# Giovannibriglia/ContinuousBayesianNetwork

Hardware: AMD Instinct MI355X
Metric: marginal queries/sec + achieved HBM GB/s, 20-node d=32 DAG, 65k-batch VE (higher is better)
Workload: dtype f32; 1 GPU; chain20_d32: BayesianNetwork.infer target X19, evidence on the other 19 nodes, N_max=32; queries_per_gpu=65536, global_batch=65536, parallelism=query-shard x1

## Files before the change

### continuousbayesiannetwork_amd/_native.py

```python
from __future__ import annotations

import ctypes
import os

import torch

from . import _buildstamp

_HERE = os.path.dirname(os.path.abspath(__file__))
_DEFAULT_LIB = os.path.join(_HERE, "libcbn_amd.so")


def lib_path() -> str:
    alt = os.environ.get("CBN_LIB_PATH")
    if alt and os.environ.get("CBN_DIAG") == "1":
        return alt
    return _DEFAULT_LIB


LIB_PATH = lib_path()

ABI_VERSION = 5
CBN_MAX_PARENTS = 8
CBN_MAX_DIRECT_PARENTS = 32
# ... 118 lines not shown
    "cbn_plan_max_words": (ctypes.c_int32, [ctypes.c_void_p]),
    "cbn_plan_run_fold": (ctypes.c_int, [ctypes.c_void_p, ctypes.c_int64, ctypes.c_void_p, ctypes.c_int32,
                                         ctypes.c_void_p, ctypes.c_void_p, ctypes.c_void_p, ctypes.c_int64,
                                         ctypes.c_void_p, ctypes.c_int32, ctypes.c_int32, ctypes.c_void_p]),
    "cbn_plan_run_argmax": (ctypes.c_int, [ctypes.c_void_p, ctypes.c_int64, ctypes.c_void_p, ctypes.c_int32,
                                           ctypes.c_void_p, ctypes.c_void_p, ctypes.c_void_p, ctypes.c_void_p,
                                           ctypes.c_void_p, ctypes.c_int32, ctypes.c_void_p]),
    "cbn_plan_argmax_scratch": (ctypes.c_int64, [ctypes.c_void_p, ctypes.c_int64]),
    "cbn_row_argmax": (ctypes.c_int, [ctypes.c_void_p, ctypes.c_int64, ctypes.c_int32, ctypes.c_void_p,
                                      ctypes.c_void_p, ctypes.c_void_p, ctypes.c_void_p, ctypes.c_void_p]),
    "cbn_plan_create_param": (ctypes.c_int, [ctypes.POINTER(ParamFactor), ctypes.c_int32, ctypes.c_int32,
                                             ctypes.POINTER(ctypes.c_void_p)]),
    "cbn_param_eval": (ctypes.c_int, [ctypes.POINTER(ParamModel), ctypes.c_void_p, ctypes.c_int64, ctypes.c_int32,
                                      ctypes.c_void_p, ctypes.c_int32, ctypes.c_void_p, ctypes.c_void_p]),
    "cbn_hash_build": (ctypes.c_int, [ctypes.c_void_p, ctypes.c_void_p, ctypes.c_int64, ctypes.c_void_p,
                                      ctypes.c_void_p, ctypes.c_int64, ctypes.c_void_p]),
    "cbn_cpd_ref_eval": (ctypes.c_int, [ctypes.POINTER(CpdRef), ctypes.c_void_p, ctypes.c_int64, ctypes.c_void_p,
                                        ctypes.c_void_p]),
    "cbn_plan_create_direct": (ctypes.c_int, [ctypes.POINTER(DirectFactor), ctypes.c_int32, ctypes.c_int32,
                                              ctypes.POINTER(ctypes.c_void_p)]),
}
CBN_RUN_BUILD_TABLES = 1
CBN_RUN_TIMED = 2
CBN_RUN_TWO_PASS = 4
CBN_RUN_RAW = 8
CBN_E_LIMIT = -3
CBN_E_UNSUPPORTED = -4
CBN_E_TIMEOUT = -5
CBN_PLAN_FAST, CBN_PLAN_LDS, CBN_PLAN_PAIRED, CBN_PLAN_STAGED = 1, 2, 4, 8
CBN_PLAN_FUSED, CBN_PLAN_PARAMETRIC, CBN_PLAN_VPL2, CBN_PLAN_DIRECT = 16, 32, 64, 128
CBN_PLAN_COLS = 256
CBN_PLAN_SLOTS = 512
CBN_PLAN_ARGMAX = 1024
CBN_E_ARG = -1

EXPORTED_SYMBOLS = tuple(_SIGNATURES)

_lib = None


class NativeError(RuntimeError):
    pass


def _check_stamp(path: str, digest: str) -> None:
    got = _buildstamp.read_stamp(path)
    if got != digest:
        raise NativeError(
            f"{path} was not built from this tree's sources (stamp {got or 'missing'} != {digest[:16]}...): "
            "rebuild it with `python -c 'import __graft_entry__ as g; g.build()'`")


def load() -> ctypes.CDLL:
    global _lib
    if _lib is None:
        if not os.path.exists(LIB_PATH):
            raise NativeError(
                f"{LIB_PATH} is missing: build it with `python -c 'import __graft_entry__ as g; g.build()'` "
                "(no CPU fallback exists for the HIP inference path)")
        if LIB_PATH == _DEFAULT_LIB:
            _check_stamp(LIB_PATH, _buildstamp.lib_digest())
        lib = ctypes.CDLL(LIB_PATH)
        for name, (res, args) in _SIGNATURES.items():
            fn = getattr(lib, name)
            fn.restype = res
            fn.argtypes = args
# ... 53 lines not shown
```

### continuousbayesiannetwork_amd/csrc/cbn_infer.hip

```cpp

#include <hip/hip_runtime.h>

#include <algorithm>
#include <cstdarg>
#include <cstdint>
#include <cstdio>
#include <cstdlib>
#include <cstring>
#include <string>
#include <type_traits>
#include <vector>

#include <unistd.h>

#include "cbn_internal.h"

using namespace cbn;

namespace {
thread_local std::string g_err;
}

namespace {
const bool g_diag = [] {
// ... 247 lines not shown
__device__ __forceinline__ void store_wt(__amdgpu_buffer_rsrc_t r, int off, float4 v) {
    u32x4_t x = {__float_as_uint(v.x), __float_as_uint(v.y), __float_as_uint(v.z), __float_as_uint(v.w)};
#ifndef CBN_STORE_AUX
#define CBN_STORE_AUX 16
#endif
    __builtin_amdgcn_raw_buffer_store_b128(x, r, off, 0, CBN_STORE_AUX);
}

__device__ __forceinline__ int4 sload_int4(const void* p) {
    const cint_t* q = reinterpret_cast<const cint_t*>(reinterpret_cast<uintptr_t>(p));
    return make_int4(q[0], q[1], q[2], q[3]);
}

constexpr int kChunkBytes = kWave * 16;
template <int K>
__device__ __forceinline__ void lds_dma_group(const float4* gp, float4* lp) {
    __builtin_amdgcn_global_load_lds((gbl_void_t*)gp, (lds_void_t*)lp, 16, 0, 0);
    if (K > 1) __builtin_amdgcn_global_load_lds((gbl_void_t*)gp, (lds_void_t*)lp, 16, kChunkBytes, 0);
    if (K > 2) __builtin_amdgcn_global_load_lds((gbl_void_t*)gp, (lds_void_t*)lp, 16, 2 * kChunkBytes, 0);
    if (K > 3) __builtin_amdgcn_global_load_lds((gbl_void_t*)gp, (lds_void_t*)lp, 16, 3 * kChunkBytes, 0);
}
__device__ __forceinline__ void lds_dma_segment(const float4* gl, float4* lds, int a, int b) {
    const float4* gp = gl + a * kWave;
    float4* lp = lds + a * kWave;
    int n = b - a;
    for (; n >= 4; n -= 4, gp += 4 * kWave, lp += 4 * kWave) lds_dma_group<4>(gp, lp);
    if (n & 2) {
        lds_dma_group<2>(gp, lp);
        gp += 2 * kWave;
        lp += 2 * kWave;
    }
    if (n & 1) lds_dma_group<1>(gp, lp);
}
__device__ __forceinline__ void lds_dma_copy(const float* __restrict__ g, float4* lds, int n4,
                                             int nw = kQueryThreads / kWave) {
    const int lane = threadIdx.x & (kWave - 1);
    const int wave = __builtin_amdgcn_readfirstlane(threadIdx.x / kWave);
    const int nchunk = (n4 + kWave - 1) / kWave;
    const int run = (nchunk + nw - 1) / nw;
    const int r0 = wave * run;
    const int len = nchunk - r0 < run ? nchunk - r0 : run;
    if (len <= 0 || !CBN_OK_OR(n4 > 0 && wave < nw, 0)) return;
    int start = r0 + (int)(blockIdx.x % (unsigned)nchunk);
    if (start >= nchunk) start -= nchunk;
    const int over = start + len - nchunk;
    const int tail = n4 & (kWave - 1);
    const float4* gl = reinterpret_cast<const float4*>(g) + lane;
    const bool masked = over >= 0 && tail != 0;
    lds_dma_segment(gl, lds, start, (over >= 0 ? nchunk : start + len) - (masked ? 1 : 0));
    if (masked && lane < tail) lds_dma_group<1>(gl + (nchunk - 1) * kWave, lds + (nchunk - 1) * kWave);
    if (over > 0) lds_dma_segment(gl, lds, 0, over);
}

__global__ void k_cpd_scatter(const int32_t* __restrict__ cell, const float* __restrict__ prob,
                              long long n_rows, float* __restrict__ cpd) {
    for (long long r = blockIdx.x * (long long)blockDim.x + threadIdx.x; r < n_rows;
         r += (long long)gridDim.x * blockDim.x)
        cpd[cell[r]] = prob[r];
}

__global__ void k_cpd_normalize(float* __restrict__ cpd, long long n_pcells, int card) {
    for (long long c = blockIdx.x * (long long)blockDim.x + threadIdx.x; c < n_pcells;
         c += (long long)gridDim.x * blockDim.x) {
        float* row = cpd + c * card;
        double s = 0.0;
        for (int v = 0; v < card; ++v) s += (double)row[v];
        const float den = (float)s + 1e-10f;
        for (int v = 0; v < card; ++v) row[v] = row[v] / den;
    }
}

__global__ void k_cpd_eval(const float* __restrict__ cpd, int n_cols, ColPtrs cols,
                           const float* __restrict__ pts, long long n_pts, float* __restrict__ out) {
    for (long long i = blockIdx.x * (long long)blockDim.x + threadIdx.x; i < n_pts;
         i += (long long)gridDim.x * blockDim.x) {
        long long off = 0;
// ... 1124 lines not shown
#pragma unroll
            for (int i = 0; i < NV; ++i) acc0[i] = acc[i];
        }
        round_epilogue<VPL, MODE>(acc, col, l, L, valid, valid, q, N, out, maxv, lmax, !first, fq, am);
        __builtin_amdgcn_s_waitcnt(0xC07F);
        __builtin_amdgcn_wave_barrier();
        if (first) CBN_STAMP(6);
        first = false;
    }
    CBN_STAMP(7);
    if (MODE == kModeMax || MODE == kModeRaw) publish_block_max(lmax, wmax, max_out, n_max, lane, wid, tid, nthr);
    if (MODE == kModeFused) {
        maxv = fused_block_max(lmax, wmax, sync, epoch, max_out, lane, wid, nthr CBN_STAMP_ARG);
        if (fq0 >= 0) store_row_div<VPL>(out + fq0 * N, col, acc0, maxv);
        if (fq >= 0) store_row_div<VPL>(out + fq * N, col, acc, maxv);
        CBN_STAMP(10);
    }
}

constexpr int kSR = 256;
constexpr int kSQ = 128;
constexpr int kSU = 4;

struct FoldJob {
    float* rows;
    const unsigned* words;
    long long n4;
    long long chunk;
    int n_words;
};
constexpr int kFoldK = 2;
constexpr int kFoldW = 4;

template <int MODE>
__global__ void __launch_bounds__(kQueryThreads)
k_query_staged(const float* __restrict__ gimage, int image_floats, int rec_off, int nf, int zero_off, long long Q,
               long long per, unsigned* __restrict__ sync, unsigned epoch, const unsigned* __restrict__ max_in,
               int n_max, unsigned* __restrict__ max_out, float* __restrict__ out, FoldJob fold,
               FPtrsT<kFastPtrsSmall> fp, ArgmaxOut am) {
    CBN_STAMP_INIT;
    constexpr int N = 32;
    extern __shared__ __attribute__((aligned(16))) float4 smem4[];
    float* simg = reinterpret_cast<float*>(smem4);
    const int T = (nf + 2) >> 1;
    const int S = (T + 1) >> 1;
    const int nsl = 4 * (S + 1);
    int* offs = reinterpret_cast<int*>(simg + image_floats);
    float* wmax = reinterpret_cast<float*>(offs + 2 * kSR * nsl);
    const int tid = threadIdx.x;
    const int lane = tid & (kWave - 1);
    const int wid = __builtin_amdgcn_readfirstlane(tid / kWave);
    const long long q0 = (long long)blockIdx.x * per;
    const long long q1 = q0 + per < Q ? q0 + per : Q;
    const int nunits = nf * (kSR / kSQ);
    const FastRec* grec = reinterpret_cast<const FastRec*>(gimage + rec_off);
    const int one_off = zero_off + 64;

    float x[kSU][2] = {};
    auto stage_load = [&](long long qr, auto ksu, int gw, int GW) {
        constexpr int KSU = decltype(ksu)::value;
        uintptr_t pk[KSU];
#pragma unroll
        for (int k = 0; k < KSU; ++k) {
            const int u = gw + k * GW;
            pk[k] = reinterpret_cast<uintptr_t>(fp.p[((u / (kSR / kSQ)) & 31) * kFastObs]);
        }
#pragma unroll
        for (int k = 0; k < KSU; ++k) {
            const int u = gw + k * GW;
            if (u < nunits) {
                const float* col = reinterpret_cast<const float*>(pk[k] & ~(kTagMore | kTagNone));
#pragma unroll
                for (int h = 0; h < 2; ++h) {
                    const long long q = qr + (u % (kSR / kSQ)) * kSQ + h * kWave + lane;
                    x[k][h] = gload(col, (pk[k] & kTagNone) ? 0 : (q < q1 ? q : q0));
                }
            }
        }
    };
    auto stage_store = [&](long long qr, int buf, auto ksu, int gw, int GW) {
        constexpr int KSU = decltype(ksu)::value;
        int* ob = offs + buf * kSR * nsl;
        int4 rk[KSU];
#pragma unroll
        for (int k = 0; k < KSU; ++k) {
            const int u = gw + k * GW;
            rk[k] = sload_int4(grec + (u < nunits ? u / (kSR / kSQ) : 0));
        }
#pragma unroll
        for (int k = 0; k < KSU; ++k) {
            const int u = gw + k * GW;
// ... 19 lines not shown
                        if (n_obs > 1) {
                            const long long q = qr + ql;
#pragma unroll
                            for (int p = 1; p < kFastObs; ++p)
                                if (p < n_obs) xs[p] = gload(fp.p[f * kFastObs + p], q < q1 ? q : q0);
                        }
                        int row = 0;
                        bool ok = true;
#pragma unroll
                        for (int p = 0; p < kFastObs; ++p) {
                            if (p < n_obs) {
                                const int card = r.card[p] & (kDenseBit - 1);
                                const float xv = xs[p];
                                int i;
                                if (r.card[p] & kDenseBit) {
                                    i = (int)xv;
                                    i = (xv >= 0.f && xv < (float)card && (float)i == xv) ? i : -1;
                                } else {
                                    i = bsearch_eq(gimage + r.dom_off[p], card, xv);
                                }
                                ok &= i >= 0;
                                row = row * card + (i < 0 ? 0 : i);
                            }
                        }
                        o = ok ? r.table_off + row * 64 : zoff;
                    }
                    ob[ql * nsl + f + ((ql >> 1) & 1)] = o;
                }
            }
        }
    };

    long long qr = q0;
#ifndef CBN_ABL_NODMA
    lds_dma_copy(gimage, smem4, image_floats / 4);
#endif
#ifndef CBN_ABL_NOSTAGE
    if (qr < q1) stage_load(qr, std::integral_constant<int, kSU>{}, wid, kQueryThreads / kWave);
#endif
    CBN_STAMP(1);
    if (tid < kSR) {
        const int d = (tid >> 1) & 1;
        for (int j = 0; j < nsl; ++j) {
            const int f = j - d;
            if (f < 0 || f >= nf) {
                const int o = one_off + (f & 1) * 32;
                offs[tid * nsl + j] = o;
                offs[kSR * nsl + tid * nsl + j] = o;
            }
        }
    }
    if (qr < q1)
        stage_store(qr, 0, std::integral_constant<int, kSU>{}, wid, kQueryThreads / kWave);
    CBN_STAMP(2);
    __syncthreads();
    CBN_STAMP(3);
    float4 fv[kFoldK];
    unsigned fw[kFoldW];
    const long long fb = (long long)blockIdx.x * fold.chunk;
    const long long fe = fb + fold.chunk < fold.n4 ? fb + fold.chunk : fold.n4;
    if (MODE == kModeRaw && fold.rows) {
        const float4* r4 = reinterpret_cast<const float4*>(fold.rows);
#pragma unroll
        for (int k = 0; k < kFoldK; ++k) {
            const long long i = fb + tid + k * kQueryThreads;
            fv[k] = i < fe ? r4[i] : make_float4(0.f, 0.f, 0.f, 0.f);
        }
#pragma unroll
        for (int k = 0; k < kFoldW; ++k) {
            const int w = lane + k * kWave;
            fw[k] = w < fold.n_words ? fold.words[w] : 0u;
        }
    }

    const int qi = lane >> 2;
    const int l = lane & 3;
    const int h0 = qi & 1;
    const int clo = (l + 4 * h0) * 4, chi = (l + 4 * (h0 ^ 1)) * 4;
    float lmax = 0.f;
    float maxv = 1.f;
    if (MODE == kModeWrite) maxv = batch_max(max_in, n_max, max_out, lane, tid);
    float acc[8];
    long long fq = -1;
    int buf = 0;
    const bool wt_raw = MODE == kModeRaw && fold.rows != nullptr;
    const __amdgpu_buffer_rsrc_t orsrc =
        rows_rsrc((MODE == kModeFused || wt_raw) ? out + q0 * N : nullptr,
                  (MODE == kModeFused || wt_raw) ? (q1 - q0) * (long long)(N * 4) : 0);
    for (; qr < q1; qr += kSR, buf ^= 1) {
        const long long qn = qr + kSR;
        if (MODE != kModeFused && qn < q1) stage_load(qn, std::integral_constant<int, kSU>{}, wid, kQueryThreads / kWave);
        const int ql = wid * 16 + qi;
        const long long q = qr + ql;
        const int* my = offs + buf * kSR * nsl + ql * nsl;
#pragma unroll
        for (int i = 0; i < 8; ++i) acc[i] = 1.f;
        auto mul_step = [&](const float4& r0, const float4& r1, const float4& r2, const float4& r3) {
            acc[0] *= r0.x; acc[1] *= r0.y; acc[2] *= r0.z; acc[3] *= r0.w;
            acc[4] *= r1.x; acc[5] *= r1.y; acc[6] *= r1.z; acc[7] *= r1.w;
            acc[0] *= r2.x; acc[1] *= r2.y; acc[2] *= r2.z; acc[3] *= r2.w;
            acc[4] *= r3.x; acc[5] *= r3.y; acc[6] *= r3.z; acc[7] *= r3.w;
        };
        auto load_step = [&](int oa, int ob, float4& r0, float4& r1, float4& r2, float4& r3) {
            r0 = *reinterpret_cast<const float4*>(simg + oa + clo);
            r1 = *reinterpret_cast<const float4*>(simg + oa + chi);
            r2 = *reinterpret_cast<const float4*>(simg + ob + clo);
            r3 = *reinterpret_cast<const float4*>(simg + ob + chi);
        };
        typedef float vf4 __attribute__((ext_vector_type(4)));
        typedef const volatile __attribute__((address_space(3))) vf4 lds_vf4;
        auto vld = [&](int o) {
            const vf4 v = *(lds_vf4*)(simg + o);
            return make_float4(v.x, v.y, v.z, v.w);
        };
        auto vload_step = [&](int oa, int ob, float4& r0, float4& r1, float4& r2, float4& r3) {
            r0 = vld(oa + clo);
            r1 = vld(oa + chi);
            r2 = vld(ob + clo);
            r3 = vld(ob + chi);
        };
        float4 A0, A1, A2, A3, B0, B1, B2, B3;
        int4 on = *reinterpret_cast<const int4*>(my);
        vload_step(on.x, on.y, A0, A1, A2, A3);
        vload_step(on.z, on.w, B0, B1, B2, B3);
// ... 12 lines not shown
            mul_step(A0, A1, A2, A3);
            load_step(on.x, on.y, A0, A1, A2, A3);
            mul_step(B0, B1, B2, B3);
            load_step(on.z, on.w, B0, B1, B2, B3);
            on = *reinterpret_cast<const int4*>(my + 4 * min(sp + 2, S));
        }
#endif
        CBN_STAMP(5);
        if (MODE == kModeArgmax) {
            const int colv[2] = {clo, chi};
            argmax_store<2>(acc, colv, l, 4, q < q1, q, am);
        }
        if (q < q1) {
            if (MODE == kModeFused) fq = q;
            if (MODE == kModeRaw && wt_raw) {
                const int ob = (int)(q - q0) * (N * 4);
                store_wt(orsrc, ob + clo * 4, make_float4(acc[0], acc[1], acc[2], acc[3]));
                store_wt(orsrc, ob + chi * 4, make_float4(acc[4], acc[5], acc[6], acc[7]));
            } else if (MODE == kModeWrite || MODE == kModeRaw) {
                const float dv = MODE == kModeWrite ? maxv : 1.f;
                float* o = out + q * N;
                *reinterpret_cast<float4*>(o + clo) = MODE == kModeWrite
                    ? make_float4(acc[0] / dv, acc[1] / dv, acc[2] / dv, acc[3] / dv)
                    : make_float4(acc[0], acc[1], acc[2], acc[3]);
                *reinterpret_cast<float4*>(o + chi) = MODE == kModeWrite
                    ? make_float4(acc[4] / dv, acc[5] / dv, acc[6] / dv, acc[7] / dv)
                    : make_float4(acc[4], acc[5], acc[6], acc[7]);
            }
            if (MODE != kModeWrite && MODE != kModeArgmax)
#pragma unroll
                for (int i = 0; i < 8; ++i) lmax = fmaxf(lmax, acc[i]);
        }
        if (MODE != kModeFused && qn < q1) {
            stage_store(qn, buf ^ 1, std::integral_constant<int, kSU>{}, wid, kQueryThreads / kWave);
            __syncthreads();
        }
    }
    CBN_STAMP(6);
    if (MODE == kModeRaw && fold.rows) {
        unsigned m = 0;
#pragma unroll
        for (int k = 0; k < kFoldW; ++k) m = max(m, fw[k]);
        m = wave_max_u(m);
        const double y = 1.0 / (double)__uint_as_float(m);
        float4* r4 = reinterpret_cast<float4*>(fold.rows);
        const __amdgpu_buffer_rsrc_t frsrc = rows_rsrc(fold.rows + fb * 4, fe > fb ? (fe - fb) * 16 : 0);
#pragma unroll
        for (int k = 0; k < kFoldK; ++k) {
            const long long i = fb + tid + k * kQueryThreads;
            if (i < fe)
                store_wt(frsrc, (int)(i - fb) * 16,
                         make_float4((float)((double)fv[k].x * y), (float)((double)fv[k].y * y),
                                     (float)((double)fv[k].z * y), (float)((double)fv[k].w * y)));
        }
        for (long long i = fb + tid + kFoldK * kQueryThreads; i < fe; i += kQueryThreads) {
            const float4 v = r4[i];
            r4[i] = make_float4((float)((double)v.x * y), (float)((double)v.y * y), (float)((double)v.z * y),
                                (float)((double)v.w * y));
        }
    }
    if (MODE == kModeMax || MODE == kModeRaw) publish_block_max(lmax, wmax, max_out, n_max, lane, wid, tid, kQueryThreads);
    if (MODE == kModeFused) {
        lmax = wave_max_nonneg(lmax);
        if (lane == 0) wmax[wid] = lmax;
        __syncthreads();
        CBN_STAMP(7);
        if (wid == 0) {
            const float bm = wave_max_nonneg(lane < kQueryThreads / kWave ? wmax[lane] : 0.f);
#ifdef CBN_ABL_NOBAR
            const unsigned gm = __float_as_uint(bm);
#else
            const unsigned gm = slot_barrier_max(sync, epoch, bm);
#endif
            if (lane == 0) {
                wmax[0] = __uint_as_float(gm);
                if (blockIdx.x == 0 && max_out) *max_out = gm;
            }
        }
        CBN_STAMP(8);
        __syncthreads();
        CBN_STAMP(9);
        maxv = wmax[0];
        if (fq >= 0) {
            const double y = 1.0 / (double)maxv;
            float o[8];
#pragma unroll
            for (int i = 0; i < 8; ++i) o[i] = (float)((double)acc[i] * y);
            const int ob = (int)(fq - q0) * (N * 4);
            store_wt(orsrc, ob + clo * 4, make_float4(o[0], o[1], o[2], o[3]));
            store_wt(orsrc, ob + chi * 4, make_float4(o[4], o[5], o[6], o[7]));
        }
        CBN_STAMP(10);
        CBN_CLOCK_END;
    }
}

__device__ __forceinline__ unsigned max_words(const unsigned* __restrict__ w, int n) {
    const int lane = threadIdx.x & (kWave - 1);
    unsigned m = 0;
    int i = lane;
    for (; i + 15 * kWave < n; i += 16 * kWave) {
        unsigned t[16];
#pragma unroll
        for (int k = 0; k < 16; ++k) t[k] = w[i + k * kWave];
#pragma unroll
        for (int k = 0; k < 16; ++k) m = max(m, t[k]);
    }
    for (; i + 3 * kWave < n; i += 4 * kWave) {
        unsigned t[4];
#pragma unroll
        for (int k = 0; k < 4; ++k) t[k] = w[i + k * kWave];
#pragma unroll
        for (int k = 0; k < 4; ++k) m = max(m, t[k]);
    }
    for (; i < n; i += kWave) m = max(m, w[i]);
    return wave_max_u(m);
}

__device__ __forceinline__ float4 div4(float4 v, float m) {
    v.x = v.x / m;
    v.y = v.y / m;
    v.z = v.z / m;
    v.w = v.w / m;
    return v;
}

template <int U>
// ... 160 lines not shown
}

size_t slots_lds_bytes(long long lds_tab_floats, int ns, int nf, int QB) {
    const size_t nf4 = (size_t)((nf + 3) & ~3);
    const size_t SQ = (size_t)slots_sidx_stride(kQueryThreads / QB);
    size_t b = (size_t)lds_tab_floats * 4 + (size_t)ns * sizeof(QSlot) + (size_t)nf * sizeof(ColRec) +
               (size_t)((ns + 1) & ~1) * sizeof(void*) + ((((size_t)ns * SQ + 7) & ~size_t(7)) * 2) +
               (size_t)QB * nf4 * 4 + (kQueryThreads / kWave) * 4 + 64;
    return (b + 15) & ~size_t(15);
}

template <int VPL, bool LDS, int MODE, int NP>
void launch_fast_np(const cbn_plan* p, unsigned blocks, hipStream_t s, const EvPtrs& ev, long long Q, int L,
                    unsigned epoch, const unsigned* max_in, int n_max, unsigned* max_out, float* out,
                    const ArgmaxOut& am) {
    hipLaunchKernelGGL((k_query_fast<VPL, LDS, MODE, NP>), dim3(blocks), dim3(kQueryThreads), p->fast_lds_bytes, s,
                       p->rec_off, p->nf, p->ns, p->d_image, p->image_floats, fast_ptrs<NP>(p, ev), Q,
                       (Q + blocks - 1) / blocks, p->N, p->RS, L, p->paired ? 1 : 0, p->d_sync, epoch, max_in, n_max,
                       max_out, out, p->lds_tab_floats, p->lds_tab_mask[0], p->lds_tab_mask[1], am);
}

template <int VPL, bool LDS, int MODE>
void launch_fast_k(const cbn_plan* p, unsigned blocks, hipStream_t s, const EvPtrs& ev, long long Q, int L,
                   unsigned epoch, const unsigned* max_in, int n_max, unsigned* max_out, float* out,
                   const FoldJob* fold = nullptr, const ArgmaxOut* amp = nullptr) {
    const ArgmaxOut am = amp ? *amp : ArgmaxOut{nullptr, nullptr, nullptr, nullptr};
    if (p->staged) {
        FoldJob fj;
        memset(&fj, 0, sizeof(fj));
        if (fold && fold->rows && fold->n4 > 0) {
            fj = *fold;
            fj.chunk = (fj.n4 + blocks - 1) / blocks;
        }
        hipLaunchKernelGGL((k_query_staged<MODE>), dim3(blocks), dim3(kQueryThreads), p->staged_lds_bytes, s,
                           p->d_image, p->image_floats, p->rec_off + p->prefix * kRecFloats, p->nf - p->prefix,
                           p->zero_off, Q, (Q + blocks - 1) / blocks, p->d_sync, epoch, max_in, n_max, max_out, out,
                           fj, fast_ptrs<kFastPtrsSmall>(p, ev, p->prefix), am);
        return;
    }
    if (p->slots) {
        const int QBs = kQueryThreads / L;
        long long per = (Q + blocks - 1) / blocks;
        int coal = per > 2LL * QBs && !diag_env("CBN_SLOTS_NO_COAL") ? 1 : 0;
        if (diag_env("CBN_SLOTS_COAL")) coal = 1;
        for (int i = 0; i < p->ns; ++i) coal &= (reinterpret_cast<uintptr_t>(ev.p[i]) & 15) == 0 ? 1 : 0;
        if (coal) per = (per + 3) & ~3LL;
        hipLaunchKernelGGL((k_query_slots<VPL, MODE>), dim3(blocks), dim3(kQueryThreads), p->fast_lds_bytes, s, p->nf,
                           p->ns, p->d_image, p->rec_off + p->nf * kRecFloats, p->d_crec, slot_ptrs(p, ev), Q, per,
                           p->N, L, p->d_sync, epoch, max_in, n_max, max_out, out, p->lds_tab_floats,
                           p->lds_tab_mask[0], p->lds_tab_mask[1], coal, am);
        return;
    }
    if (p->cols) {
        auto k = (p->ns + L - 1) / L <= 16 ? k_query_cols<VPL, LDS, MODE, 16> : k_query_cols<VPL, LDS, MODE, 40>;
        hipLaunchKernelGGL(k, dim3(blocks), dim3(kQueryThreads), p->fast_lds_bytes, s,
                           p->rec_off, p->nf, p->ns, p->d_image, p->image_floats, slot_ptrs(p, ev), Q,
                           (Q + blocks - 1) / blocks, p->N, p->RS, L, p->d_sync, epoch, max_in, n_max, max_out, out,
                           p->lds_tab_floats, p->d_crec, am);
        return;
    }
    if (p->nf * kFastObs <= kFastPtrsSmall)
        launch_fast_np<VPL, LDS, MODE, kFastPtrsSmall>(p, blocks, s, ev, Q, L, epoch, max_in, n_max, max_out, out, am);
    else
        launch_fast_np<VPL, LDS, MODE, kFastPtrs>(p, blocks, s, ev, Q, L, epoch, max_in, n_max, max_out, out, am);
}

template <int VPL, bool LDS, int MODE>
const void* fast_kernel_fn(int nf, bool cols = false, int slots_per_lane = 0) {
    if (cols)
        return slots_per_lane <= 16 ? reinterpret_cast<const void*>(&k_query_cols<VPL, LDS, MODE, 16>)
// ... 549 lines not shown
            }
        }
    }
    int vpl = 0, Lf = 0;
    if (fast) {
        int want = 2;
        if (const char* e = diag_env("CBN_FAST_VPL")) want = atoi(e);
        for (int c : {2, 1}) {
            if (c > want || (N / 4) % c) continue;
            const int Lc = N / (4 * c);
            if (Lc <= kWave && (kWave % Lc) == 0) { vpl = c; Lf = Lc; break; }
        }
        fast = vpl > 0;
    }
    if (fast) {
        const int nf4 = (n_factors + 3) & ~3;
        const size_t side = (size_t)kFastPtrs * sizeof(void*) +
                            (size_t)(kQueryThreads / kWave) * (kWave / Lf) * nf4 * 4 + (kQueryThreads / kWave) * 4 + 64;
        const bool lds_ok = img_bytes + side <= (size_t)kLdsBudget;
        if (!lds_ok && P->use_lds) fast = false;
        if (!P->use_lds && (size_t)P->lds_tab_floats * 4 + (size_t)n_factors * kRecFloats * 4 + side > (size_t)kLdsBudget)
            fast = false;
        if (fast) {
            P->fast = true;
            P->vpl = vpl;
            P->paired = paired && vpl == 2 && P->use_lds;
            const int st_T = (n_factors - P->prefix + 2) >> 1, st_S = (st_T + 1) >> 1;
            const size_t st_bytes =
                img_bytes + (size_t)2 * kSR * (4 * (st_S + 1)) * 4 + (kQueryThreads / kWave) * 4 + 64;
            if (P->paired && (n_factors - P->prefix) * kFastObs <= kFastPtrsSmall && st_bytes <= (size_t)kLdsBudget &&
                !diag_env("CBN_NO_STAGED")) {
                P->staged = true;
                P->staged_lds_bytes = (st_bytes + 15) & ~size_t(15);
                for (const void* fn : {reinterpret_cast<const void*>(&k_query_staged<kModeMax>),
                                       reinterpret_cast<const void*>(&k_query_staged<kModeWrite>),
                                       reinterpret_cast<const void*>(&k_query_staged<kModeFused>),
                                       reinterpret_cast<const void*>(&k_query_staged<kModeRaw>),
                                       reinterpret_cast<const void*>(&k_query_staged<kModeArgmax>)})
                    (void)hipFuncSetAttribute(fn, hipFuncAttributeMaxDynamicSharedMemorySize, kLdsBudget);
            }
            P->fast_lds_bytes =
                ((P->use_lds ? img_bytes : (size_t)P->lds_tab_floats * 4 + (size_t)n_factors * kRecFloats * 4) + side +
                 15) & ~size_t(15);
            if (!P->staged && !P->paired && Lf <= 2 && ns <= kFastPtrsSmall && n_factors <= kWave &&
                !diag_env("CBN_NO_COLS")) {
                std::vector<ColRec> cr;
                bool ok_c = col_records(recs, slot_card, ns, RS, P->use_lds, lds_mask, cr);
                const size_t QBc = (size_t)kQueryThreads / Lf;
                const size_t cols_bytes =
                    ((P->use_lds ? img_bytes
                                 : (size_t)P->lds_tab_floats * 4 + ((size_t)n_factors * kRecFloats + (size_t)ns * 4) * 4) +
                     (size_t)((ns + 1) & ~1) * sizeof(void*) + (((size_t)ns * QBc + 1) & ~size_t(1)) * 2 +
                     (kQueryThreads / kWave) * 4 + 64 + 16 + (size_t)N * 4 + 15) & ~size_t(15);
                if (ok_c && cols_bytes <= (size_t)kLdsBudget) {
                    ok_c = hipMalloc(&P->d_crec, sizeof(ColRec) * n_factors) == hipSuccess &&
                           hipMemcpy(P->d_crec, cr.data(), sizeof(ColRec) * n_factors, hipMemcpyHostToDevice) ==
                               hipSuccess;
                    if (!ok_c) {
                        cbn_plan_destroy(P);
                        return set_err(CBN_E_HIP, "cbn_plan_create: column records upload failed");
                    }
                    P->cols = true;
                    P->fast_lds_bytes = cols_bytes;
                }
            }
            if (!P->staged && !P->paired && !P->cols && !P->use_lds && Lf > 2 && ns <= kFastPtrsSmall &&
                n_factors <= 128 && !diag_env("CBN_NO_SLOTS")) {
                std::vector<ColRec> cr;
                bool ok_s = col_records(recs, slot_card, ns, RS, false, lds_mask, cr);
                for (int f = 0; f < n_factors; ++f)
                    ok_s = ok_s && (long long)recs[f].table_off + (long long)fac[f].rows * RS < (1LL << 31);
                const size_t sb = slots_lds_bytes(P->lds_tab_floats, ns, n_factors, kQueryThreads / Lf);
                if (ok_s && sb <= (size_t)kLdsBudget) {
                    if (hipMalloc(&P->d_crec, sizeof(ColRec) * n_factors) != hipSuccess ||
                        hipMemcpy(P->d_crec, cr.data(), sizeof(ColRec) * n_factors, hipMemcpyHostToDevice) !=
                            hipSuccess) {
                        cbn_plan_destroy(P);
                        return set_err(CBN_E_HIP, "cbn_plan_create: slot records upload failed");
                    }
                    P->slots = true;
                    P->fast_lds_bytes = sb;
                }
            }
            P->fast_blocks_per_cu = 2 * P->fast_lds_bytes <= (size_t)kLdsBudget ? 2 : 1;
            if (P->slots)
                if (const char* e = diag_env("CBN_SLOTS_BPC")) P->fast_blocks_per_cu = atoi(e) == 2 ? 2 : 1;
            P->max_slots = std::min(num_cu() * P->fast_blocks_per_cu, kMaxSlots);
            if (hipMemcpy(P->d_image + rec_off, recs.data(), sizeof(FastRec) * n_factors, hipMemcpyHostToDevice) !=
                    hipSuccess ||
                (ns > 0 && hipMemcpy(P->d_image + rec_off + (long long)n_factors * kRecFloats, qs.data(),
                                     sizeof(QSlot) * ns, hipMemcpyHostToDevice) != hipSuccess)) {
                cbn_plan_destroy(P);
                return set_err(CBN_E_HIP, "cbn_plan_create: fast records upload failed");
            }
            if (!diag_env("CBN_NO_FUSED")) {
                allow_fast_lds<1, true, kModeFused>(kLdsBudget);
                allow_fast_lds<2, true, kModeFused>(kLdsBudget);
                allow_fast_lds<1, false, kModeFused>(kLdsBudget);
                allow_fast_lds<2, false, kModeFused>(kLdsBudget);
                int nb = 0;
                const int spl = (ns + Lf - 1) / Lf;
                const void* fn = with_variant(P, [&](auto v, auto lds) {
                    if (P->staged) return reinterpret_cast<const void*>(&k_query_staged<kModeFused>);
                    if (P->slots) return reinterpret_cast<const void*>(&k_query_slots<v.value, kModeFused>);
                    return fast_kernel_fn<v.value, lds.value, kModeFused>(n_factors, P->cols, spl);
                });
                const size_t lb = P->staged ? P->staged_lds_bytes : P->fast_lds_bytes;
                if (hipOccupancyMaxActiveBlocksPerMultiprocessor(&nb, fn, kQueryThreads, lb) == hipSuccess && nb >= 1)
                    P->fused_ok = true;
            }
        }
    }
    if (!P->staged && P->prefix) {
        P->prefix = 0;
        P->prefix_rows = 0;
    }
    allow_lds<4, true, false>(kLdsBudget); allow_lds<4, true, true>(kLdsBudget);
    allow_lds<1, true, false>(kLdsBudget); allow_lds<1, true, true>(kLdsBudget);
    allow_lds<4, false, false>(kLdsBudget); allow_lds<4, false, true>(kLdsBudget);
    allow_lds<1, false, false>(kLdsBudget); allow_lds<1, false, true>(kLdsBudget);
    if (!P->d_fac || !P->d_slots || !P->d_build || !P->d_image || !P->d_sync) {
        cbn_plan_destroy(P);
        return set_err(CBN_E_HIP, "cbn_plan_create: internal error, plan buffer missing");
    }
    *plan = P;
    return CBN_OK;
}

int cbn_plan_destroy(cbn_plan* plan) {
    if (!plan) return CBN_OK;
    for (int i = 0; i < cbn_plan::kRing; ++i)
        for (int k = 0; k < 3; ++k)
            if (plan->ev[i][k]) (void)hipEventDestroy(plan->ev[i][k]);
    if (plan->d_fac) (void)hipFree(plan->d_fac);
    if (plan->d_crec) (void)hipFree(plan->d_crec);
    if (plan->d_slots) (void)hipFree(plan->d_slots);
// ... 200 lines not shown
    EvPtrs ev;
    CBN_TRY(pack_evidence(plan, evidence, n_evidence, n_queries, ev));
    return launch_mode<kModeArgmax>(plan, n_queries, ev, nullptr, 0, nullptr, nullptr, s, nullptr, &am);
}

int cbn_plan_status(cbn_plan* plan, int32_t* status) {
    if (!plan || !status) return set_err(CBN_E_ARG, "cbn_plan_status: bad arguments");
    unsigned v = 0;
    HIP_TRY(hipMemcpy(&v, plan->d_sync + 2, sizeof(unsigned), hipMemcpyDeviceToHost));
    *status = (int32_t)v;
    if (plan->h_status) __atomic_store_n(plan->h_status, 0u, __ATOMIC_RELEASE);
    return CBN_OK;
}

int cbn_plan_check(cbn_plan* plan) {
    if (!plan) return set_err(CBN_E_ARG, "cbn_plan_check: null plan");
    if (plan->h_status && __atomic_load_n(plan->h_status, __ATOMIC_ACQUIRE)) {
        __atomic_store_n(plan->h_status, 0u, __ATOMIC_RELEASE);
        return set_err(CBN_E_TIMEOUT, "a single-launch call of this plan timed out in its grid barrier (another "
                                      "stream held CUs its blocks needed): its rows are NaN");
    }
    return CBN_OK;
}

int64_t cbn_plan_fused_capacity(const cbn_plan* plan) { return plan ? fused_capacity(plan) : 0; }

int32_t cbn_plan_flags(const cbn_plan* plan) {
    if (!plan) return 0;
    return (plan->fast ? CBN_PLAN_FAST : 0) | (plan->use_lds ? CBN_PLAN_LDS : 0) |
           (plan->paired ? CBN_PLAN_PAIRED : 0) | (plan->staged ? CBN_PLAN_STAGED : 0) |
           (plan->fused_ok ? CBN_PLAN_FUSED : 0) | (plan->param ? CBN_PLAN_PARAMETRIC : 0) |
           (plan->vpl == 2 ? CBN_PLAN_VPL2 : 0) | (plan->direct ? CBN_PLAN_DIRECT : 0) |
           (plan->cols ? CBN_PLAN_COLS : 0) | (plan->slots ? CBN_PLAN_SLOTS : 0) |
           (argmax_native(plan) ? CBN_PLAN_ARGMAX : 0);
}

int32_t cbn_plan_max_words(const cbn_plan* plan) {
    if (plan && plan->param) return param_max_words(plan->param);
    if (plan && plan->direct) return direct_max_words(plan->direct);
    return plan && plan->fast ? plan->max_slots : 0;
}

int cbn_scale(float* out, int64_t n, const uint32_t* max_bits, int32_t n_max, void* stream) {
    if (n < 0 || n_max < 1 || (n > 0 && (!out || !max_bits))) return set_err(CBN_E_ARG, "cbn_scale: bad arguments");
    if (n == 0) return CBN_OK;
    if (reinterpret_cast<uintptr_t>(out) % 16) return set_err(CBN_E_ARG, "cbn_scale: out must be 16-B aligned");
    return launch_scale(out, (long long)n, max_bits, (int)n_max, nullptr, reinterpret_cast<hipStream_t>(stream));
}

namespace {
int scale_blocks_per_cu() {
    static int v = [] {
        const char* e = diag_env("CBN_SCALE_BLOCKS_PER_CU");
        const int x = e ? atoi(e) : 0;
        return x >= 1 && x <= 16 ? x : 1;
    }();
    return v;
}
}

int cbn_scale_batch(float* const* outs, const int64_t* n_elems, int32_t n_batches, const uint32_t* max_bits,
                    int32_t n_max, void* stream) {
    if (n_batches < 0 || n_batches > kScaleBatch || n_max < 1 || (n_batches > 0 && (!outs || !n_elems || !max_bits)))
        return set_err(CBN_E_ARG, "cbn_scale_batch: bad arguments (at most %d batches)", kScaleBatch);
    if (n_batches == 0) return CBN_OK;
    ScaleBatch sb;
    memset(&sb, 0, sizeof(sb));
// ... 46 lines not shown
```

### continuousbayesiannetwork_amd/csrc/cbn_internal.h

```cpp
#ifndef CBN_INTERNAL_H
#define CBN_INTERNAL_H

#include <hip/hip_runtime.h>

#include <cstdint>

#include "../../include/cbn_amd.h"

namespace cbn {

constexpr int kWave = 64;
constexpr int kLdsBudget = 160 * 1024;
constexpr int kFastPtrs = 416;

constexpr int kSyncLine = 32;
constexpr int kHostStatusWordOff = 8;
constexpr int kOneWordOff = 12;
constexpr int kMaxSlots = 1024;
constexpr int kSlotWordOff = kSyncLine;
constexpr int kMaxWordOff = kSlotWordOff + 2 * kMaxSlots;
constexpr int kSyncWords = kMaxWordOff + kMaxSlots;

struct DevFactor;
struct QSlot;
// ... 16 lines not shown
               uint32_t* max_bits, float* out, int32_t flags, hipStream_t s);
int direct_build_consts(DirectPlan* dp, hipStream_t s);
void direct_destroy(DirectPlan* dp);
int direct_max_words(const DirectPlan* dp);

}

struct cbn_plan {
    int nf = 0;
    int ns = 0;
    int N = 0;
    int vec = 1;
    int L = 1;
    int CH = 1;
    cbn::DevFactor* d_fac = nullptr;
    int* d_crec = nullptr;
    cbn::QSlot* d_slots = nullptr;
    cbn::BuildItem* d_build = nullptr;
    int n_build = 0;
    int build_units = 0;
    float* d_image = nullptr;
    unsigned* d_sync = nullptr;
    bool fast = false;
    int fast_slot[cbn::kFastPtrs];
    static constexpr int kRing = 512;
    hipEvent_t ev[kRing][3] = {};
    int ev_n = 0;
    int rec_off = 0;
    int RS = 1;
    int vpl = 1;
    bool paired = false;
    bool staged = false;
    size_t staged_lds_bytes = 0;
    bool cols = false;
    bool slots = false;
    int zero_off = -1;
    int prefix = 0;
    int prefix_offs[9] = {};
    int prefix_rows = 0;
    unsigned* h_status = nullptr;
    unsigned fused_epoch = 0;
    bool fused_ok = false;
    size_t fast_lds_bytes = 0;
    int lds_tab_floats = 0;
    unsigned long long lds_tab_mask[2] = {0, 0};
    int fast_blocks_per_cu = 1;
    int max_slots = 0;
    int image_floats = 0;
    int table_floats = 0;
    bool use_lds = false;
    size_t lds_bytes = 0;
    int blocks_per_cu = 1;
    cbn::ParamPlan* param = nullptr;
    cbn::DirectPlan* direct = nullptr;
};

#endif
```

### include/cbn_amd.h

```cpp
#ifndef CBN_AMD_H
#define CBN_AMD_H

#include <stdint.h>

#ifdef __cplusplus
extern "C" {
#endif

#define CBN_AMD_ABI_VERSION 5

#define CBN_MAX_PARENTS 8
#define CBN_MAX_EVIDENCE 256

#define CBN_OK 0
#define CBN_E_ARG -1
#define CBN_E_HIP -2
#define CBN_E_LIMIT -3
#define CBN_E_UNSUPPORTED -4
#define CBN_E_TIMEOUT -5

#define CBN_FACTOR_SCALAR 0
#define CBN_FACTOR_SHARED 1
#define CBN_FACTOR_QUERY 2

// ... 83 lines not shown

int cbn_scale(float* out, int64_t n, const uint32_t* max_bits, int32_t n_max, void* stream);
int cbn_scale_batch(float* const* outs, const int64_t* n_elems, int32_t n_batches, const uint32_t* max_bits,
                    int32_t n_max, void* stream);
int cbn_plan_run_fold(cbn_plan* plan, int64_t n_queries, const float* const* evidence, int32_t n_evidence,
                      uint32_t* max_bits, float* out, float* fold_rows, int64_t fold_n_elems,
                      const uint32_t* fold_words, int32_t fold_n_words, int32_t flags, void* stream);
int cbn_plan_status(cbn_plan* plan, int32_t* status);


int cbn_plan_run_argmax(cbn_plan* plan, int64_t n_queries, const float* const* evidence, int32_t n_evidence,
                        const float* target_values , int32_t* index,
                        float* value , float* row_max , float* scratch, int32_t flags,
                        void* stream);

int64_t cbn_plan_argmax_scratch(const cbn_plan* plan, int64_t n_queries);

int cbn_row_argmax(const float* rows, int64_t n_rows, int32_t n_cols, const float* target_values, int32_t* index,
                   float* value, float* row_max, void* stream);

int cbn_plan_check(cbn_plan* plan);

#define CBN_PLAN_FAST 1
#define CBN_PLAN_LDS 2
#define CBN_PLAN_PAIRED 4
#define CBN_PLAN_STAGED 8
#define CBN_PLAN_FUSED 16
#define CBN_PLAN_PARAMETRIC 32
#define CBN_PLAN_VPL2 64
#define CBN_PLAN_DIRECT 128
#define CBN_PLAN_COLS 256
#define CBN_PLAN_SLOTS 512
#define CBN_PLAN_ARGMAX 1024
int32_t cbn_plan_flags(const cbn_plan* plan);

int cbn_debug_flag_timeout(cbn_plan* plan);

int32_t cbn_diag_enabled(void);

int cbn_plan_timing(cbn_plan* plan, int32_t* n_timed, float* avg_max_ms, float* avg_write_ms);

#define CBN_MAX_LAYERS 4
#define CBN_MAX_WIDTH 32
#define CBN_MAX_MODEL_LAYERS 64
#define CBN_MAX_MODEL_WIDTH 256
#define CBN_FAMILY_GAUSS 1
#define CBN_FAMILY_LOGISTIC 2
#define CBN_ACT_TANH 1
#define CBN_ACT_RELU 2
#define CBN_ACT_SIGMOID 3
#define CBN_ACT_LEAKYRELU 4
#define CBN_ACT_GELU 5
#define CBN_ACT_ELU 6
#define CBN_INPUT_FREE -1
#define CBN_INPUT_ONE -2

typedef struct cbn_param_model {
    int32_t family;
    int32_t n_layers;
    int32_t width[CBN_MAX_LAYERS + 1];
    int32_t act;
    const float* weights;
    float scale;
    float norm;
    const int32_t* widths;
} cbn_param_model;
// ... 21 lines not shown
```

Before: 7.220 billion queries/s.

## Add dense single-observation fast path to staged query kernel

Adds a specialised staged kernel for the common case where every factor has at most one dense observed parent. The per-factor table offset and cardinality are packed host-side into the pointer slots, so the kernel reads them directly instead of walking the FastRec image from global memory during staging. The modulo in the LDS DMA rotation is also replaced by a precomputed magic-number reciprocal. This doubles the number of kernel instantiations and repurposes a pointer slot and the rec_off argument, with the original general path kept behind an environment switch.

```diff
diff --git a/continuousbayesiannetwork_amd/_native.py b/continuousbayesiannetwork_amd/_native.py
--- a/continuousbayesiannetwork_amd/_native.py
+++ b/continuousbayesiannetwork_amd/_native.py
@@ -174,6 +174,7 @@
 CBN_PLAN_COLS = 256
 CBN_PLAN_SLOTS = 512
 CBN_PLAN_ARGMAX = 1024
+CBN_PLAN_DENSE1 = 2048
 CBN_E_ARG = -1
 
 EXPORTED_SYMBOLS = tuple(_SIGNATURES)
diff --git a/continuousbayesiannetwork_amd/csrc/cbn_infer.hip b/continuousbayesiannetwork_amd/csrc/cbn_infer.hip
--- a/continuousbayesiannetwork_amd/csrc/cbn_infer.hip
+++ b/continuousbayesiannetwork_amd/csrc/cbn_infer.hip
@@ -303,8 +303,9 @@
     }
     if (n & 1) lds_dma_group<1>(gp, lp);
 }
+template <bool ROT_MAGIC = false>
 __device__ __forceinline__ void lds_dma_copy(const float* __restrict__ g, float4* lds, int n4,
-                                             int nw = kQueryThreads / kWave) {
+                                             int nw = kQueryThreads / kWave, unsigned rot_magic = 0) {
     const int lane = threadIdx.x & (kWave - 1);
     const int wave = __builtin_amdgcn_readfirstlane(threadIdx.x / kWave);
     const int nchunk = (n4 + kWave - 1) / kWave;
@@ -312,7 +313,14 @@
     const int r0 = wave * run;
     const int len = nchunk - r0 < run ? nchunk - r0 : run;
     if (len <= 0 || !CBN_OK_OR(n4 > 0 && wave < nw, 0)) return;
-    int start = r0 + (int)(blockIdx.x % (unsigned)nchunk);
+    unsigned rot;
+    if (ROT_MAGIC) {
+        const unsigned b = blockIdx.x;
+        rot = b - (unsigned)(((unsigned long long)b * rot_magic) >> 32) * (unsigned)nchunk;
+    } else {
+        rot = blockIdx.x % (unsigned)nchunk;
+    }
+    int start = r0 + (int)rot;
     if (start >= nchunk) start -= nchunk;
     const int over = start + len - nchunk;
     const int tail = n4 & (kWave - 1);
@@ -1503,12 +1511,23 @@
 constexpr int kFoldK = 2;
 constexpr int kFoldW = 4;
 
-template <int MODE>
-__global__ void __launch_bounds__(kQueryThreads)
-k_query_staged(const float* __restrict__ gimage, int image_floats, int rec_off, int nf, int zero_off, long long Q,
-               long long per, unsigned* __restrict__ sync, unsigned epoch, const unsigned* __restrict__ max_in,
-               int n_max, unsigned* __restrict__ max_out, float* __restrict__ out, FoldJob fold,
-               FPtrsT<kFastPtrsSmall> fp, ArgmaxOut am) {
+struct alignas(16) DenseEnt {
+    uintptr_t col;
+    int table_off;
+    int card;
+};
+static_assert(sizeof(DenseEnt) == 2 * sizeof(const float*), "DenseEnt = the first two pointer slots of a factor");
+__host__ __device__ inline unsigned dma_rot_magic(int n4) {
+    const unsigned nchunk = (unsigned)((n4 + kWave - 1) / kWave);
+    return nchunk ? (unsigned)(0x100000000ull / nchunk) + 1u : 0u;
+}
+
+template <int MODE, bool DENSE1>
+__device__ __forceinline__ void
+query_staged(const float* __restrict__ gimage, int image_floats, int rec_off, int nf, int zero_off, long long Q,
+             long long per, unsigned* __restrict__ sync, unsigned epoch, const unsigned* __restrict__ max_in,
+             int n_max, unsigned* __restrict__ max_out, float* __restrict__ out, const FoldJob& fold,
+             const FPtrsT<kFastPtrsSmall>& fp, const ArgmaxOut& am) {
     CBN_STAMP_INIT;
     constexpr int N = 32;
     extern __shared__ __attribute__((aligned(16))) float4 smem4[];
@@ -1528,6 +1547,52 @@
     const int one_off = zero_off + 64;
 
     float x[kSU][2] = {};
+    constexpr int kGW = kQueryThreads / kWave;
+    auto dense_ent = [&](int k) {
+        const int u = wid + k * kGW;
+        DenseEnt e;
+        __builtin_memcpy(&e, &fp.p[((u / (kSR / kSQ)) & 31) * kFastObs], sizeof(e));
+        return e;
+    };
+    auto dense_load = [&](long long qr, const DenseEnt (&ent)[kSU]) {
+#pragma unroll
+        for (int k = 0; k < kSU; ++k) {
+            const int u = wid + k * kGW;
+            const float* col = reinterpret_cast<const float*>(ent[k].col & ~(kTagMore | kTagNone));
+            const long long keep = (ent[k].col & kTagNone) ? 0 : -1;
+#pragma unroll
+            for (int h = 0; h < 2; ++h) {
+                const long long q = qr + (u % (kSR / kSQ)) * kSQ + h * kWave + lane;
+                x[k][h] = gload(col, (q < q1 ? q : q0) & keep);
+            }
+        }
+    };
+    auto dense_store = [&](int buf, const DenseEnt (&ent)[kSU]) {
+        int* ob = offs + buf * kSR * nsl;
+#pragma unroll
+        for (int k = 0; k < kSU; ++k) {
+            const int u = wid + k * kGW;
+            const int f = u / (kSR / kSQ);
+            const int zoff = zero_off + (f & 1) * 32;
+            const bool none = (ent[k].col & kTagNone) != 0;
+            const int toff = ent[k].table_off, card = ent[k].card;
+            int o[2];
+#pragma unroll
+            for (int h = 0; h < 2; ++h) {
+                const float xv = x[k][h];
+                const int i = (int)xv;
+                const bool ok = xv >= 0.f && xv < (float)card && (float)i == xv;
+                o[h] = none ? toff : (ok ? toff + i * 64 : zoff);
+            }
+            if (u < nunits) {
+#pragma unroll
+                for (int h = 0; h < 2; ++h) {
+                    const int ql = (u % (kSR / kSQ)) * kSQ + h * kWave + lane;
+                    ob[ql * nsl + f + ((ql >> 1) & 1)] = o[h];
+                }
+            }
+        }
+    };
     auto stage_load = [&](long long qr, auto ksu, int gw, int GW) {
         constexpr int KSU = decltype(ksu)::value;
         uintptr_t pk[KSU];
@@ -1613,11 +1678,24 @@
     };
 
     long long qr = q0;
+    DenseEnt ent0[kSU] = {};
+    if constexpr (DENSE1) {
+#pragma unroll
+        for (int k = 0; k < kSU; ++k) ent0[k] = dense_ent(k);
+    }
 #ifndef CBN_ABL_NODMA
-    lds_dma_copy(gimage, smem4, image_floats / 4);
+    if constexpr (DENSE1)
+        lds_dma_copy<true>(gimage, smem4, image_floats / 4, kGW, (unsigned)rec_off);
+    else
+        lds_dma_copy(gimage, smem4, image_floats / 4);
 #endif
 #ifndef CBN_ABL_NOSTAGE
-    if (qr < q1) stage_load(qr, std::integral_constant<int, kSU>{}, wid, kQueryThreads / kWave);
+    if (qr < q1) {
+        if constexpr (DENSE1)
+            dense_load(qr, ent0);
+        else
+            stage_load(qr, std::integral_constant<int, kSU>{}, wid, kQueryThreads / kWave);
+    }
 #endif
     CBN_STAMP(1);
     if (tid < kSR) {
@@ -1631,8 +1709,12 @@
             }
         }
     }
-    if (qr < q1)
-        stage_store(qr, 0, std::integral_constant<int, kSU>{}, wid, kQueryThreads / kWave);
+    if (qr < q1) {
+        if constexpr (DENSE1)
+            dense_store(0, ent0);
+        else
+            stage_store(qr, 0, std::integral_constant<int, kSU>{}, wid, kQueryThreads / kWave);
+    }
     CBN_STAMP(2);
     __syncthreads();
     CBN_STAMP(3);
@@ -1670,7 +1752,16 @@
                   (MODE == kModeFused || wt_raw) ? (q1 - q0) * (long long)(N * 4) : 0);
     for (; qr < q1; qr += kSR, buf ^= 1) {
         const long long qn = qr + kSR;
-        if (MODE != kModeFused && qn < q1) stage_load(qn, std::integral_constant<int, kSU>{}, wid, kQueryThreads / kWave);
+        if (MODE != kModeFused && qn < q1) {
+            if constexpr (DENSE1) {
+                DenseEnt ent[kSU];
+#pragma unroll
+                for (int k = 0; k < kSU; ++k) ent[k] = dense_ent(k);
+                dense_load(qn, ent);
+            } else {
+                stage_load(qn, std::integral_constant<int, kSU>{}, wid, kQueryThreads / kWave);
+            }
+        }
         const int ql = wid * 16 + qi;
         const long long q = qr + ql;
         const int* my = offs + buf * kSR * nsl + ql * nsl;
@@ -1749,7 +1840,14 @@
                 for (int i = 0; i < 8; ++i) lmax = fmaxf(lmax, acc[i]);
         }
         if (MODE != kModeFused && qn < q1) {
-            stage_store(qn, buf ^ 1, std::integral_constant<int, kSU>{}, wid, kQueryThreads / kWave);
+            if constexpr (DENSE1) {
+                DenseEnt ent[kSU];
+#pragma unroll
+                for (int k = 0; k < kSU; ++k) ent[k] = dense_ent(k);
+                dense_store(buf ^ 1, ent);
+            } else {
+                stage_store(qn, buf ^ 1, std::integral_constant<int, kSU>{}, wid, kQueryThreads / kWave);
+            }
             __syncthreads();
         }
     }
@@ -1810,6 +1908,25 @@
         CBN_STAMP(10);
         CBN_CLOCK_END;
     }
+}
+
+template <int MODE>
+__global__ void __launch_bounds__(kQueryThreads)
+k_query_staged(const float* __restrict__ gimage, int image_floats, unsigned rot_magic, int nf, int zero_off, long long Q,
+               long long per, unsigned* __restrict__ sync, unsigned epoch, const unsigned* __restrict__ max_in,
+               int n_max, unsigned* __restrict__ max_out, float* __restrict__ out, FoldJob fold,
+               FPtrsT<kFastPtrsSmall> fp, ArgmaxOut am) {
+    query_staged<MODE, true>(gimage, image_floats, (int)rot_magic, nf, zero_off, Q, per, sync, epoch, max_in, n_max,
+                             max_out, out, fold, fp, am);
+}
+template <int MODE>
+__global__ void __launch_bounds__(kQueryThreads)
+k_query_staged_gen(const float* __restrict__ gimage, int image_floats, int rec_off, int nf, int zero_off, long long Q,
+                   long long per, unsigned* __restrict__ sync, unsigned epoch, const unsigned* __restrict__ max_in,
+                   int n_max, unsigned* __restrict__ max_out, float* __restrict__ out, FoldJob fold,
+                   FPtrsT<kFastPtrsSmall> fp, ArgmaxOut am) {
+    query_staged<MODE, false>(gimage, image_floats, rec_off, nf, zero_off, Q, per, sync, epoch, max_in, n_max, max_out,
+                              out, fold, fp, am);
 }
 
 __device__ __forceinline__ unsigned max_words(const unsigned* __restrict__ w, int n) {
@@ -2036,10 +2153,20 @@
             fj = *fold;
             fj.chunk = (fj.n4 + blocks - 1) / blocks;
         }
-        hipLaunchKernelGGL((k_query_staged<MODE>), dim3(blocks), dim3(kQueryThreads), p->staged_lds_bytes, s,
+        FPtrsT<kFastPtrsSmall> fp = fast_ptrs<kFastPtrsSmall>(p, ev, p->prefix);
+        if (p->dense1) {
+            for (int f = 0; f < p->nf - p->prefix; ++f)
+                fp.p[f * kFastObs + 1] = reinterpret_cast<const float*>(static_cast<uintptr_t>(p->dense_rec[f]));
+            hipLaunchKernelGGL((k_query_staged<MODE>), dim3(blocks), dim3(kQueryThreads), p->staged_lds_bytes, s,
+                               p->d_image, p->image_floats, dma_rot_magic(p->image_floats / 4), p->nf - p->prefix,
+                               p->zero_off, Q, (Q + blocks - 1) / blocks, p->d_sync, epoch, max_in, n_max, max_out, out,
+                               fj, fp, am);
+            return;
+        }
+        hipLaunchKernelGGL((k_query_staged_gen<MODE>), dim3(blocks), dim3(kQueryThreads), p->staged_lds_bytes, s,
                            p->d_image, p->image_floats, p->rec_off + p->prefix * kRecFloats, p->nf - p->prefix,
                            p->zero_off, Q, (Q + blocks - 1) / blocks, p->d_sync, epoch, max_in, n_max, max_out, out,
-                           fj, fast_ptrs<kFastPtrsSmall>(p, ev, p->prefix), am);
+                           fj, fp, am);
         return;
     }
     if (p->slots) {
@@ -2655,11 +2782,24 @@
                 !diag_env("CBN_NO_STAGED")) {
                 P->staged = true;
                 P->staged_lds_bytes = (st_bytes + 15) & ~size_t(15);
+                bool dense1 = !diag_env("CBN_STAGED_GENERAL");
+                for (int f = P->prefix; f < n_factors; ++f)
+                    dense1 = dense1 && (recs[f].n_obs == 0 || (recs[f].n_obs == 1 && (recs[f].card[0] & kDenseBit)));
+                P->dense1 = dense1;
+                for (int f = P->prefix; f < n_factors && dense1; ++f)
+                    P->dense_rec[f - P->prefix] =
+                        (unsigned long long)(unsigned)recs[f].table_off |
+                        ((unsigned long long)(unsigned)(recs[f].n_obs ? recs[f].card[0] & (kDenseBit - 1) : 0) << 32);
                 for (const void* fn : {reinterpret_cast<const void*>(&k_query_staged<kModeMax>),
                                        reinterpret_cast<const void*>(&k_query_staged<kModeWrite>),
                                        reinterpret_cast<const void*>(&k_query_staged<kModeFused>),
                                        reinterpret_cast<const void*>(&k_query_staged<kModeRaw>),
-                                       reinterpret_cast<const void*>(&k_query_staged<kModeArgmax>)})
+                                       reinterpret_cast<const void*>(&k_query_staged<kModeArgmax>),
+                                       reinterpret_cast<const void*>(&k_query_staged_gen<kModeMax>),
+                                       reinterpret_cast<const void*>(&k_query_staged_gen<kModeWrite>),
+                                       reinterpret_cast<const void*>(&k_query_staged_gen<kModeFused>),
+                                       reinterpret_cast<const void*>(&k_query_staged_gen<kModeRaw>),
+                                       reinterpret_cast<const void*>(&k_query_staged_gen<kModeArgmax>)})
                     (void)hipFuncSetAttribute(fn, hipFuncAttributeMaxDynamicSharedMemorySize, kLdsBudget);
             }
             P->fast_lds_bytes =
@@ -2724,7 +2864,9 @@
                 int nb = 0;
                 const int spl = (ns + Lf - 1) / Lf;
                 const void* fn = with_variant(P, [&](auto v, auto lds) {
-                    if (P->staged) return reinterpret_cast<const void*>(&k_query_staged<kModeFused>);
+                    if (P->staged)
+                        return P->dense1 ? reinterpret_cast<const void*>(&k_query_staged<kModeFused>)
+                                         : reinterpret_cast<const void*>(&k_query_staged_gen<kModeFused>);
                     if (P->slots) return reinterpret_cast<const void*>(&k_query_slots<v.value, kModeFused>);
                     return fast_kernel_fn<v.value, lds.value, kModeFused>(n_factors, P->cols, spl);
                 });
@@ -2991,7 +3133,7 @@
            (plan->fused_ok ? CBN_PLAN_FUSED : 0) | (plan->param ? CBN_PLAN_PARAMETRIC : 0) |
            (plan->vpl == 2 ? CBN_PLAN_VPL2 : 0) | (plan->direct ? CBN_PLAN_DIRECT : 0) |
            (plan->cols ? CBN_PLAN_COLS : 0) | (plan->slots ? CBN_PLAN_SLOTS : 0) |
-           (argmax_native(plan) ? CBN_PLAN_ARGMAX : 0);
+           (argmax_native(plan) ? CBN_PLAN_ARGMAX : 0) | (plan->staged && plan->dense1 ? CBN_PLAN_DENSE1 : 0);
 }
 
 int32_t cbn_plan_max_words(const cbn_plan* plan) {
diff --git a/continuousbayesiannetwork_amd/csrc/cbn_internal.h b/continuousbayesiannetwork_amd/csrc/cbn_internal.h
--- a/continuousbayesiannetwork_amd/csrc/cbn_internal.h
+++ b/continuousbayesiannetwork_amd/csrc/cbn_internal.h
@@ -72,6 +72,8 @@
     bool paired = false;
     bool staged = false;
     size_t staged_lds_bytes = 0;
+    bool dense1 = false;
+    unsigned long long dense_rec[32] = {};
     bool cols = false;
     bool slots = false;
     int zero_off = -1;
diff --git a/include/cbn_amd.h b/include/cbn_amd.h
--- a/include/cbn_amd.h
+++ b/include/cbn_amd.h
@@ -139,6 +139,7 @@
 #define CBN_PLAN_COLS 256
 #define CBN_PLAN_SLOTS 512
 #define CBN_PLAN_ARGMAX 1024
+#define CBN_PLAN_DENSE1 2048
 int32_t cbn_plan_flags(const cbn_plan* plan);
 
 int cbn_debug_flag_timeout(cbn_plan* plan);
```

Result: slower. 6.808 billion queries/s (-5.7%).
